# samuel-vitorino/lm.rs

Measured on AMD Instinct MI355X. Metric: decode tok/s + %HBM-roofline, Llama-3.2-1B Q8_0 @1/2/4/8 MI355X vs CPU ref, higher is better.
Workload: dtype int8xint8->int32, f32 combine; 1 GPU; llama-3.2-1b Q8_0 (gs=128) greedy decode, 5-token synthetic prompt then 3164 tokens, batch 1; parallelism=single GPU, image_bytes=1274634496

## Files before the change

lm.rs_amd/csrc/lmrs_kernels.hip:

```cpp
#include <hip/hip_ext.h>
#include <mutex>
#include <map>
#include <set>
#include <tuple>
#include <utility>

#include "lmrs_device_math.h"
#include "lmrs_kernels.h"
#include "lmrs_stage.h"

namespace lmrs {

constexpr int kBlock = 256;
constexpr int kGS = 128;


constexpr int kMaxP = 16;

template <int NP>
__device__ __forceinline__ void rmsnorm_inplace(float4 (&v)[NP], const float4 (&wv)[NP], int n, float eps,
                                                int add_unit, float* scratch) {
    const int t = threadIdx.x;
    const int P = (n + 1023) >> 10;
    const int JP = (n >> 3) + 4;
// ... 1155 lines not shown
    }
    for (int j = tid; j < (ROT ? 0 : half); j += kBlock) {
        float2 cs;
        if constexpr (PRE) cs = pre.cs; else if constexpr (TAG) cs = cs_tag; else cs = *reinterpret_cast<const float2*>(a.rope + ((size_t)pos * half + j) * 2);
        const float fcr = cs.x, fci = cs.y;
        const float q0 = TAG ? q[j] : PRE ? pre.q0 : ld_f32<COH>(a.q + h * HS + j), q1 = TAG ? q[j + half] : PRE ? pre.q1 : ld_f32<COH>(a.q + h * HS + j + half);
        const float2 rq = rope_rotate(q0, q1, fcr, fci);
        q[j] = rq.x; q[j + half] = rq.y;
        const float k0 = TAG ? kn[j] : PRE ? pre.k0 : ld_f32<COH>(a.k_raw + kvh * HS + j), k1 = TAG ? kn[j + half] : PRE ? pre.k1 : ld_f32<COH>(a.k_raw + kvh * HS + j + half);
        const float2 rk = rope_rotate(k0, k1, fcr, fci);
        kn[j] = rk.x; kn[j + half] = rk.y;
        k_store_pair(kT, S, pos, j, half, rk.x, rk.y);
        if constexpr (COH) {
            vn[j] = ld_f32<true>(vbase + (size_t)pos * kv_dim + j);
            vn[j + half] = ld_f32<true>(vbase + (size_t)pos * kv_dim + j + half);
        }
    }
    if (!TAG || HS / 4 > KG || T > kBlock) asm volatile("s_waitcnt vmcnt(0)" ::: "memory");
    lds_barrier();
    ATT_STAMP(2);
    if (!ROT && tc0 == pos) {
#pragma unroll
        for (int u = 0; u < KG; ++u) { const float4 t4 = reinterpret_cast<const float4*>(kn)[u]; kk[u] = f32x4v{t4.x, t4.y, t4.z, t4.w}; }
    }

    int wpos = pos;
    if constexpr (GEMMA) { const int wb = a.st->win_base; wpos = wb >= 0 ? wb : pos; }
    const float sqrt_hs = sqrtf((float)HS);
    float lmax = __uint_as_float(0xff800000u);
    auto finish_score = [&](float score, int t) __attribute__((always_inline)) {
        score = score / sqrt_hs;
        if constexpr (GEMMA) score = gemma_cap_window(score, wpos, t);
        if (t < T) { att[t] = score; lmax = fmaxf(lmax, score); }
    };
    finish_score(att_score_chain<HS, KG>(kk, krs, tc0 * 16, q, S), tid);
    for (int t0 = kBlock; t0 < T; t0 += kBlock) {
        const int t = t0 + tid, tc = t < T ? t : T - 1;
        f32x4v k0[KG];
        att_kload<KG>(k0, krs, tc * 16, 0, S);
        finish_score(att_score_chain<HS, KG>(k0, krs, tc * 16, q, S), t);
    }
    ATT_STAMP(4);
    lmax = wave64_max(lmax);
    if ((tid & 63) == 0) red[tid >> 6] = lmax;
    lds_barrier();
    const float mx = fmaxf(fmaxf(red[0], red[1]), fmaxf(red[2], red[3]));
    for (int t0 = 0; t0 < T; t0 += kBlock) {
        const int t = t0 + tid;
        const float e = expf_glibc_t(t < T ? att[t] - mx : 0.0f, etab);
        if (t < T) att[t] = e;
    }
    if (tid < 64) att[T + tid] = 0.0f;
    lds_barrier();
    if (tid < 64) {
        float sum = 0.0f;
        for (int t0 = 0; t0 < T; t0 += 64) {
            const int left = T - t0;
            sum = wave_serial_sum(sum, att[t0 + tid], left >= 64 ? 4 : (left + 15) >> 4);
        }
        if (tid == 0) red[4] = sum;
    }
    lds_barrier();
    const float sum = red[4];
    for (int t = tid; t < T; t += kBlock) att[t] = att[t] / sum;
    lds_barrier();
    ATT_STAMP(5);

    float o = 0.0f;
    for (int c = 0; c < nchunks; ++c) {
        const int t0 = c * CH, ct = (T - t0) < CH ? (T - t0) : CH;
        att_tstore<HS, NF, true>(vreg, tile, att + t0, t0, T, CH, (COH || TAG) ? pos : -1, vn);
        lds_barrier();
        if (c + 1 < nchunks) att_gload<HS, NF>(vreg, vbase, t0 + CH, T, CH, kv_dim);
        if (c == 0) ATT_STAMP(6);
        if (tid < HS) {
            o = serial_sum16<RS, false>(o, tile + tid, ct);
        }
        lds_barrier();
    }
    if (tid < HS) st_f32<COH>(a.out + h * HS + tid, o);
    ATT_STAMP(7);
}

template <int HS, bool GEMMA>
__global__ __launch_bounds__(kBlock) void attention_kernel(const AttnArgs a) {
    extern __shared__ __attribute__((aligned(16))) char smem[];
    const int h = blockIdx.x, kvh = h / (a.n_heads / a.n_kv_heads);
    ATT_STAMP(0);
    const uint64_t etab = exp2f_tab_lane();
    constexpr int half = HS / 2;
    const int j = threadIdx.x < half ? (int)threadIdx.x : 0;
    const int pos = a.st->pos;
    AttPre pre;
    pre.q0 = a.q[h * HS + j]; pre.q1 = a.q[h * HS + j + half];
    pre.k0 = a.k_raw[kvh * HS + j]; pre.k1 = a.k_raw[kvh * HS + j + half];
    pre.cs = *reinterpret_cast<const float2*>(a.rope + ((size_t)pos * half + j) * 2);
    ATT_STAMP(1);
    attention_body<HS, kAttF4, false, true, GEMMA>(a, h, pos, smem, etab, pre);
}

static size_t attention_smem(int head_size, int chunk, int seq_len) {
    return (size_t)(3 * head_size + 16 + (size_t)(chunk + 32) * (head_size + 4) + ((seq_len + 3) & ~3) + 64) * 4;
}

int attention_chunk(int head_size) {
    int ch = (16384 / head_size) & ~31;
    if (ch > 256) ch = 256;
    return ch < 32 ? 32 : ch;
}

template <int HS, bool GEMMA>
static hipError_t launch_attention_hsg(const AttnArgs& a, size_t smem, hipStream_t s) {
    allow_big_lds(reinterpret_cast<const void*>(attention_kernel<HS, GEMMA>));
    LMRS_LAUNCH_GRID((attention_kernel<HS, GEMMA>), dim3(a.n_heads), kBlock, smem, s, a);
    return hipGetLastError();
}
template <int HS>
static hipError_t launch_attention_hs(const AttnArgs& a, size_t smem, hipStream_t s) {
    return a.gemma ? launch_attention_hsg<HS, true>(a, smem, s) : launch_attention_hsg<HS, false>(a, smem, s);
}

hipError_t launch_attention(const AttnArgs& a0, hipStream_t s) {
    AttnArgs a = a0;
    a.chunk = attention_chunk(a.head_size);
    if (a.chunk * (a.head_size / 4) > kAttF4 * kBlock) return hipErrorInvalidValue;
    const size_t smem = attention_smem(a.head_size, a.chunk, a.seq_len);
    switch (a.head_size) {
        case 64: return launch_attention_hs<64>(a, smem, s);
        case 96: return launch_attention_hs<96>(a, smem, s);
        case 128: return launch_attention_hs<128>(a, smem, s);
        case 256: return launch_attention_hs<256>(a, smem, s);
        default: return hipErrorInvalidValue;
    }
}

template <int HS> struct WaveGeom {
    static constexpr int HS4 = HS / 4, ND = (HS + 63) / 64, NH2 = (HS / 2 + 63) / 64;
    static constexpr int TW = HS <= 64 ? 128 : 64;
    static constexpr int NPASS = TW / 64;
    static constexpr size_t SMEM = (size_t)(2 * HS + TW + 16) * 4 + (size_t)HS4 * TW * 16;
};
constexpr int qa_wave_T(int hs) { return hs == 64 ? 64 * 4 : ((hs == 96 || hs == 128) ? 128 : 0); }

template <int HS, bool GEMMA>
__device__ __forceinline__ void attention_wave_tag(const AttnArgs& a, const int h, const int pos, char* smem, const uint64_t etab, const AttTag& tg) {
    using W = WaveGeom<HS>;
    constexpr int HS4 = W::HS4, ND = W::ND, NH2 = W::NH2, TW = W::TW, NPASS = W::NPASS, half = HS / 2;
    const int lane = threadIdx.x & 63;
    const int kv_mul = a.n_heads / a.n_kv_heads, kvh = h / kv_mul, kv_dim = a.n_kv_heads * HS;
    const int T = pos + 1, S = a.seq_len;
    float* qs = reinterpret_cast<float*>(smem);
    float* kn = qs + HS;
    float* att = kn + HS;
    float4* kt = reinterpret_cast<float4*>(att + TW + 16);
    float* kT = att_k_head(a, kvh, HS);
    const float* vbase = a.v_cache + (size_t)a.layer * S * kv_dim + kvh * HS;
    if (a.dbg && lane == 0 && blockIdx.x == 0) a.dbg[0] = wall_clock64();

    float2 cs[NH2];
#pragma unroll
    for (int i = 0; i < NH2; ++i) { const int j = lane + 64 * i; cs[i] = *reinterpret_cast<const float2*>(a.rope + ((size_t)pos * half + (j < half ? j : 0)) * 2); }
#pragma unroll
    for (int p = 0; p < NPASS; ++p) {
        if (64 * p < pos) {
#pragma unroll
            for (int g = 0; g < HS4; ++g)
                __builtin_amdgcn_global_load_lds((const LMRS_GLOBAL void*)(kT + ((size_t)g * S + 64 * p + lane) * 4),
                                                 (__attribute__((address_space(3))) void*)(kt + g * TW + 64 * p), 16, 0, 0);
        }
    }
    float v[ND][TW];
    const __amdgpu_buffer_rsrc_t vrs = __builtin_amdgcn_make_buffer_rsrc(const_cast<float*>(vbase), 0, 0x7fffffff, 0x00020000);
    const int vrow = kv_dim * 4;
    auto vblock = [&](auto self, auto t0c) __attribute__((always_inline)) -> void {
        constexpr int t0 = decltype(t0c)::value;
        if constexpr (t0 < TW) {
            if (t0 < pos) {
#pragma unroll
                for (int u = 0; u < 16; ++u)
#pragma unroll
                    for (int i = 0; i < ND; ++i) {
                        const int d = lane + 64 * i;
                        v[i][t0 + u] = __uint_as_float(__builtin_amdgcn_raw_buffer_load_b32(vrs, (d < HS ? d : 0) * 4, (t0 + u) * vrow, 0));
                    }
                self(self, std::integral_constant<int, t0 + 16>());
            }
        }
    };
    vblock(vblock, std::integral_constant<int, 0>());
#pragma unroll
    for (int t = 0; t < TW; ++t)
#pragma unroll
        for (int i = 0; i < ND; ++i) { v[i][t] = t < pos ? v[i][t] : 0.0f; asm volatile("" : "+v"(v[i][t])); }
    if (a.dbg && lane == 0 && blockIdx.x == 0) a.dbg[1] = wall_clock64();

    unsigned long long xg[3 * ND];
    {
        const unsigned long long* gp[3 * ND];
#pragma unroll
        for (int i = 0; i < ND; ++i) { const int d = lane + 64 * i; granules_of(tg, h, kvh, HS, d < HS ? d : 0, gp + 3 * i); }
        poll_granules<3 * ND>(gp, tg, a.layer, xg);
    }
    asm volatile("s_waitcnt vmcnt(0)" ::: "memory");
    if (a.dbg && lane == 0 && blockIdx.x == 0) a.dbg[2] = wall_clock64();
    float vnew[ND];
#pragma unroll
    for (int i = 0; i < ND; ++i) {
        const int d = lane + 64 * i;
        vnew[i] = __uint_as_float((unsigned)xg[3 * i + 2]);
        if (d < HS) { qs[d] = __uint_as_float((unsigned)xg[3 * i]); kn[d] = __uint_as_float((unsigned)xg[3 * i + 1]); }
    }
#pragma unroll
    for (int i = 0; i < NH2; ++i) {
        const int j = lane + 64 * i;
        if (j < half) {
            const float2 rq = rope_rotate(qs[j], qs[j + half], cs[i].x, cs[i].y);
            qs[j] = rq.x; qs[j + half] = rq.y;
            const float2 rk = rope_rotate(kn[j], kn[j + half], cs[i].x, cs[i].y);
            k_store_pair(kT, S, pos, j, half, rk.x, rk.y);
            k_store_pair(reinterpret_cast<float*>(kt), TW, pos, j, half, rk.x, rk.y);
        }
    }
    if (a.dbg && lane == 0 && blockIdx.x == 0) a.dbg[3] = wall_clock64();

    int wpos = pos;
    if constexpr (GEMMA) { const int wb = a.st->win_base; wpos = wb >= 0 ? wb : pos; }
    const float sqrt_hs = sqrtf((float)HS), ninf = __uint_as_float(0xff800000u);
    float sc[NPASS];
    float lmax = ninf;
#pragma unroll
    for (int p = 0; p < NPASS; ++p) {
        sc[p] = ninf;
        if (64 * p < T) {
            const int t = 64 * p + lane;
            float score = tile_score<HS4>(kt + t, TW, qs) / sqrt_hs;
            if constexpr (GEMMA) score = gemma_cap_window(score, wpos, t);
            sc[p] = t < T ? score : ninf;
            lmax = fmaxf(lmax, sc[p]);
        }
    }
    if (a.dbg && lane == 0 && blockIdx.x == 0) a.dbg[4] = wall_clock64();
    const float mx = wave64_max(lmax);
    float ex[NPASS];
#pragma unroll
    for (int p = 0; p < NPASS; ++p) {
        ex[p] = 0.0f;
        if (64 * p < T) {
            const int t = 64 * p + lane;
            const float e = expf_glibc_t(t < T ? sc[p] - mx : 0.0f, etab);
            ex[p] = t < T ? e : 0.0f;
        }
    }
    float sum = 0.0f;
#pragma unroll
    for (int p = 0; p < NPASS; ++p) {
        if (64 * p < T) {
            const int left = T - 64 * p;
            sum = wave_serial_sum(sum, ex[p], left >= 64 ? 4 : (left + 15) >> 4);
        }
    }
    float ap_lane = 0.0f;
#pragma unroll
    for (int p = 0; p < NPASS; ++p) {
        if (64 * p < T) {
            const int t = 64 * p + lane;
            const float w = ex[p] / sum;
            att[t] = t < pos ? w : 0.0f;
            if ((pos >> 6) == p) ap_lane = w;
        }
    }
    const float a_pos = __builtin_bit_cast(float, __builtin_amdgcn_readlane(__builtin_bit_cast(int, ap_lane), pos & 63));
    if (a.dbg && lane == 0 && blockIdx.x == 0) a.dbg[5] = wall_clock64();
    float o[ND];
#pragma unroll
    for (int i = 0; i < ND; ++i) o[i] = 0.0f;
#pragma unroll
    for (int t0 = 0; t0 < TW; t0 += 16) {
        if (t0 < pos) {
            float4 w4[4];
#pragma unroll
            for (int u = 0; u < 4; ++u) w4[u] = reinterpret_cast<const float4*>(att)[t0 / 4 + u];
#pragma unroll
            for (int u = 0; u < 4; ++u)
#pragma unroll
                for (int i = 0; i < ND; ++i) {
                    float pr;
                    pr = w4[u].x * v[i][t0 + 4 * u + 0]; o[i] = o[i] + pr;
                    pr = w4[u].y * v[i][t0 + 4 * u + 1]; o[i] = o[i] + pr;
                    pr = w4[u].z * v[i][t0 + 4 * u + 2]; o[i] = o[i] + pr;
                    pr = w4[u].w * v[i][t0 + 4 * u + 3]; o[i] = o[i] + pr;
                }
        }
    }
#pragma unroll
    for (int i = 0; i < ND; ++i) {
        const int d = lane + 64 * i;
        const float pr = a_pos * vnew[i];
        o[i] = o[i] + pr;
        if (d < HS) a.out[h * HS + d] = o[i];
    }
    if (a.dbg && lane == 0 && blockIdx.x == 0) a.dbg[7] = wall_clock64();
}

constexpr size_t kPairSmem = (size_t)(2 * 2 * 64 + 128 + 16 + 16) * 4 + (size_t)16 * 128 * 16 + (size_t)64 * 64 * 4;
template <bool GEMMA>
__device__ __forceinline__ void attention_pair_tag(const AttnArgs& a, const int h, const int pos, char* smem, const uint64_t etab, const AttTag& tg) {
    constexpr int HS = 64, HS4 = 16, TW = 128, half = 32;
    const int lane = threadIdx.x & 63, wv = __builtin_amdgcn_readfirstlane((int)threadIdx.x >> 6);
    const bool two = pos >= 64;
    if (wv > (two ? 1 : 0)) return;
    const int tb = two ? 64 * wv : 0;
    const int kv_mul = a.n_heads / a.n_kv_heads, kvh = h / kv_mul, kv_dim = a.n_kv_heads * HS;
    const int T = pos + 1, S = a.seq_len;
    float* base = reinterpret_cast<float*>(smem);
    float* qs = base + wv * 2 * HS;
    float* kn = qs + HS;
    float* att = base + 4 * HS;
    float* red = att + TW + 16;
    float4* kt = reinterpret_cast<float4*>(red + 16);
    float* prod = reinterpret_cast<float*>(kt + HS4 * TW);
    float* kT = att_k_head(a, kvh, HS);
    const float* vbase = a.v_cache + (size_t)a.layer * S * kv_dim + kvh * HS;
    if (a.dbg && lane == 0 && wv == 0 && blockIdx.x == 0) a.dbg[0] = wall_clock64();

    const float2 cs = *reinterpret_cast<const float2*>(a.rope + ((size_t)pos * half + (lane < half ? lane : 0)) * 2);
    if (tb < pos) {
#pragma unroll
        for (int g = 0; g < HS4; ++g)
            __builtin_amdgcn_global_load_lds((const LMRS_GLOBAL void*)(kT + ((size_t)g * S + tb + lane) * 4),
                                             (__attribute__((address_space(3))) void*)(kt + g * TW + tb), 16, 0, 0);
    }
    float v[64];
    const __amdgpu_buffer_rsrc_t vrs = __builtin_amdgcn_make_buffer_rsrc(const_cast<float*>(vbase), 0, 0x7fffffff, 0x00020000);
    const int vrow = kv_dim * 4, vb0 = tb * vrow;
    auto vblock = [&](auto self, auto u0c) __attribute__((always_inline)) -> void {
        constexpr int u0 = decltype(u0c)::value;
        if constexpr (u0 < 64) {
            if (tb + u0 < pos) {
#pragma unroll
                for (int u = 0; u < 16; ++u) v[u0 + u] = __uint_as_float(__builtin_amdgcn_raw_buffer_load_b32(vrs, lane * 4, vb0 + (u0 + u) * vrow, 0));
                self(self, std::integral_constant<int, u0 + 16>());
            }
        }
    };
    vblock(vblock, std::integral_constant<int, 0>());
#pragma unroll
    for (int u = 0; u < 64; ++u) { v[u] = tb + u < pos ? v[u] : 0.0f; asm volatile("" : "+v"(v[u])); }
    if (a.dbg && lane == 0 && wv == 0 && blockIdx.x == 0) a.dbg[1] = wall_clock64();

    unsigned long long xg[3];
    {
        const unsigned long long* gp[3];
        granules_of(tg, h, kvh, HS, lane, gp);
        poll_granules<3>(gp, tg, a.layer, xg);
    }
    asm volatile("s_waitcnt vmcnt(0)" ::: "memory");
    if (a.dbg && lane == 0 && wv == 0 && blockIdx.x == 0) a.dbg[2] = wall_clock64();
    const float vnew = __uint_as_float((unsigned)xg[2]);
    qs[lane] = __uint_as_float((unsigned)xg[0]); kn[lane] = __uint_as_float((unsigned)xg[1]);
    if (lane < half) {
        const int j = lane;
        const float2 rq = rope_rotate(qs[j], qs[j + half], cs.x, cs.y);
        qs[j] = rq.x; qs[j + half] = rq.y;
        const float2 rk = rope_rotate(kn[j], kn[j + half], cs.x, cs.y);
        if (wv == 0) k_store_pair(kT, S, pos, j, half, rk.x, rk.y);
        if ((pos >> 6) == (two ? wv : 0)) k_store_pair(reinterpret_cast<float*>(kt), TW, pos, j, half, rk.x, rk.y);
    }
    if (a.dbg && lane == 0 && wv == 0 && blockIdx.x == 0) a.dbg[3] = wall_clock64();

    int wpos = pos;
    if constexpr (GEMMA) { const int wb = a.st->win_base; wpos = wb >= 0 ? wb : pos; }
    const float sqrt_hs = sqrtf((float)HS), ninf = __uint_as_float(0xff800000u);
    const int t = tb + lane;
    float sc;
    {
        float score = tile_score<HS4>(kt + t, TW, qs) / sqrt_hs;
        if constexpr (GEMMA) score = gemma_cap_window(score, wpos, t);
        sc = t < T ? score : ninf;
    }
    if (a.dbg && lane == 0 && wv == 0 && blockIdx.x == 0) a.dbg[4] = wall_clock64();
    float mx = wave64_max(sc);
    if (two) {
        if (lane == 0) red[wv] = mx;
        lds_barrier();
        mx = fmaxf(red[0], red[1]);
    }
    const float e0 = expf_glibc_t(t < T ? sc - mx : 0.0f, etab);
    const float ex = t < T ? e0 : 0.0f;
    float sum;
    if (!two) {
        sum = wave_serial_sum(0.0f, ex, (T + 15) >> 4);
    } else {
        if (wv == 0) { sum = wave_serial_sum(0.0f, ex, 4); if (lane == 0) red[2] = sum; }
        lds_barrier();
        if (wv == 1) { sum = wave_serial_sum(red[2], ex, (T - 64 + 15) >> 4); if (lane == 0) red[3] = sum; }
        lds_barrier();
        sum = red[3];
    }
    const float w = ex / sum;
    att[t] = t < pos ? w : 0.0f;
    const bool own_pos = (pos >> 6) == (two ? wv : 0);
    float a_pos = 0.0f;
    if (own_pos) a_pos = __builtin_bit_cast(float, __builtin_amdgcn_readlane(__builtin_bit_cast(int, w), pos & 63));
    if (a.dbg && lane == 0 && wv == 0 && blockIdx.x == 0) a.dbg[5] = wall_clock64();
    if (two && wv == 1) {
        if (lane == 0) red[4] = a_pos;
#pragma unroll
        for (int u0 = 0; u0 < 64; u0 += 16) {
            if (64 + u0 < pos) {
                float4 w4[4];
#pragma unroll
                for (int u = 0; u < 4; ++u) w4[u] = reinterpret_cast<const float4*>(att)[(64 + u0) / 4 + u];
#pragma unroll
                for (int u = 0; u < 4; ++u) {
                    prod[(u0 + 4 * u + 0) * HS + lane] = w4[u].x * v[u0 + 4 * u + 0];
                    prod[(u0 + 4 * u + 1) * HS + lane] = w4[u].y * v[u0 + 4 * u + 1];
                    prod[(u0 + 4 * u + 2) * HS + lane] = w4[u].z * v[u0 + 4 * u + 2];
                    prod[(u0 + 4 * u + 3) * HS + lane] = w4[u].w * v[u0 + 4 * u + 3];
                }
            }
        }
        lds_barrier();
        return;
    }
    float o = 0.0f;
#pragma unroll
    for (int u0 = 0; u0 < 64; u0 += 16) {
        if (u0 < pos) {
            float4 w4[4];
#pragma unroll
            for (int u = 0; u < 4; ++u) w4[u] = reinterpret_cast<const float4*>(att)[u0 / 4 + u];
#pragma unroll
            for (int u = 0; u < 4; ++u) {
                float pr;
                pr = w4[u].x * v[u0 + 4 * u + 0]; o = o + pr;
                pr = w4[u].y * v[u0 + 4 * u + 1]; o = o + pr;
                pr = w4[u].z * v[u0 + 4 * u + 2]; o = o + pr;
                pr = w4[u].w * v[u0 + 4 * u + 3]; o = o + pr;
            }
        }
    }
    if (two) {
        lds_barrier();
        a_pos = red[4];
#pragma unroll
        for (int u0 = 0; u0 < 64; u0 += 16) {
            if (64 + u0 < pos) {
                float pb[16];
#pragma unroll
                for (int u = 0; u < 16; ++u) pb[u] = prod[(u0 + u) * HS + lane];
#pragma unroll
                for (int u = 0; u < 16; ++u) o = o + pb[u];
            }
        }
    }
    {
        const float pr = a_pos * vnew;
        o = o + pr;
        a.out[h * HS + lane] = o;
    }
    if (a.dbg && lane == 0 && wv == 0 && blockIdx.x == 0) a.dbg[7] = wall_clock64();
}

constexpr int kMultiWaves = 4;
constexpr size_t kMultiSmem = (size_t)(kMultiWaves * 2 * 64 + 64 * kMultiWaves + 16 + 32) * 4 + (size_t)(kMultiWaves - 1) * 64 * 64 * 4;
template <bool GEMMA>
__device__ __forceinline__ void attention_multi_tag(const AttnArgs& a, const int h, const int pos, char* smem, const uint64_t etab, const AttTag& tg) {
    constexpr int HS = 64, HS4 = 16, half = 32;
    const int lane = threadIdx.x & 63, wv = __builtin_amdgcn_readfirstlane((int)threadIdx.x >> 6);
    const int nw = (pos >> 6) + 1 < kMultiWaves ? (pos >> 6) + 1 : kMultiWaves;
    if (wv >= nw) return;
    const int tb = 64 * wv, t = tb + lane;
    const int kv_mul = a.n_heads / a.n_kv_heads, kvh = h / kv_mul, kv_dim = a.n_kv_heads * HS;
    const int T = pos + 1, S = a.seq_len;
    float* base = reinterpret_cast<float*>(smem);
    float* qs = base + wv * 2 * HS;
    float* kn = qs + HS;
    float* att = base + kMultiWaves * 2 * HS;
    float* red = att + 64 * kMultiWaves + 16;
    float* prod = red + 32;
    float* kT = att_k_head(a, kvh, HS);
    const float* vbase = a.v_cache + (size_t)a.layer * S * kv_dim + kvh * HS;
    if (a.dbg && lane == 0 && wv == 0 && blockIdx.x == 0) a.dbg[0] = wall_clock64();

    const float2 cs = *reinterpret_cast<const float2*>(a.rope + ((size_t)pos * half + (lane < half ? lane : 0)) * 2);
    f32x4v kreg[HS4];
    {
        const int tk = t < S ? t : S - 1;
        if (tb < pos) {
#pragma unroll
            for (int g = 0; g < HS4; ++g) kreg[g] = *reinterpret_cast<const f32x4v*>(kT + ((size_t)g * S + tk) * 4);
        } else {
#pragma unroll
            for (int g = 0; g < HS4; ++g) kreg[g] = f32x4v{0.0f, 0.0f, 0.0f, 0.0f};
        }
    }
    float v[64];
    const __amdgpu_buffer_rsrc_t vrs = __builtin_amdgcn_make_buffer_rsrc(const_cast<float*>(vbase), 0, 0x7fffffff, 0x00020000);
    const int vrow = kv_dim * 4;
    auto vblock = [&](auto self, auto u0c) __attribute__((always_inline)) -> void {
        constexpr int u0 = decltype(u0c)::value;
        if constexpr (u0 < 64) {
            if (tb + u0 < pos) {
#pragma unroll
                for (int u = 0; u < 16; ++u) {
                    const int row = tb + u0 + u < S ? tb + u0 + u : S - 1;
                    v[u0 + u] = __uint_as_float(__builtin_amdgcn_raw_buffer_load_b32(vrs, lane * 4, row * vrow, 0));
                }
                self(self, std::integral_constant<int, u0 + 16>());
            }
        }
    };
    vblock(vblock, std::integral_constant<int, 0>());
#pragma unroll
    for (int u = 0; u < 64; ++u) { v[u] = tb + u < pos ? v[u] : 0.0f; asm volatile("" : "+v"(v[u])); }
    if (a.dbg && lane == 0 && wv == 0 && blockIdx.x == 0) a.dbg[1] = wall_clock64();

    unsigned long long xg[3];
    {
        const unsigned long long* gp[3];
        granules_of(tg, h, kvh, HS, lane, gp);
        poll_granules<3>(gp, tg, a.layer, xg);
    }
    asm volatile("s_waitcnt vmcnt(0)" ::: "memory");
    if (a.dbg && lane == 0 && wv == 0 && blockIdx.x == 0) a.dbg[2] = wall_clock64();
    const float vnew = __uint_as_float((unsigned)xg[2]);
    qs[lane] = __uint_as_float((unsigned)xg[0]); kn[lane] = __uint_as_float((unsigned)xg[1]);
    const bool own_pos = (pos >> 6) == wv;
    if (lane < half) {
        const int j = lane;
        const float2 rq = rope_rotate(qs[j], qs[j + half], cs.x, cs.y);
        qs[j] = rq.x; qs[j + half] = rq.y;
        const float2 rk = rope_rotate(kn[j], kn[j + half], cs.x, cs.y);
        kn[j] = rk.x; kn[j + half] = rk.y;
        if (wv == 0) k_store_pair(kT, S, pos, j, half, rk.x, rk.y);
    }
    if (own_pos) {
#pragma unroll
        for (int g = 0; g < HS4; ++g) {
            const float4 n4 = reinterpret_cast<const float4*>(kn)[g];
            const bool me = lane == (pos & 63);
            kreg[g][0] = me ? n4.x : kreg[g][0]; kreg[g][1] = me ? n4.y : kreg[g][1]; kreg[g][2] = me ? n4.z : kreg[g][2]; kreg[g][3] = me ? n4.w : kreg[g][3];
        }
    }
    if (a.dbg && lane == 0 && wv == 0 && blockIdx.x == 0) a.dbg[3] = wall_clock64();

    int wpos = pos;
    if constexpr (GEMMA) { const int wb = a.st->win_base; wpos = wb >= 0 ? wb : pos; }
    const float sqrt_hs = sqrtf((float)HS), ninf = __uint_as_float(0xff800000u);
    float sc;
    {
        float score = 0.0f;
#pragma unroll
        for (int g = 0; g < HS4; ++g) {
            const float4 q4 = reinterpret_cast<const float4*>(qs)[g];
            float pr;
            pr = q4.x * kreg[g][0]; score = score + pr;
            pr = q4.y * kreg[g][1]; score = score + pr;
            pr = q4.z * kreg[g][2]; score = score + pr;
            pr = q4.w * kreg[g][3]; score = score + pr;
        }
        score = score / sqrt_hs;
        if constexpr (GEMMA) score = gemma_cap_window(score, wpos, t);
        sc = t < T ? score : ninf;
    }
    if (a.dbg && lane == 0 && wv == 0 && blockIdx.x == 0) a.dbg[4] = wall_clock64();
    float mx = wave64_max(sc);
    if (nw > 1) {
        if (lane == 0) red[wv] = mx;
        lds_barrier();
        mx = red[0];
        for (int w = 1; w < nw; ++w) mx = fmaxf(mx, red[w]);
    }
    const float e0 = expf_glibc_t(t < T ? sc - mx : 0.0f, etab);
    const float ex = t < T ? e0 : 0.0f;
    float sum;
    if (nw == 1) {
        sum = wave_serial_sum(0.0f, ex, (T + 15) >> 4);
    } else {
        for (int s = 0; s < nw; ++s) {
            if (wv == s) {
                const int left = T - 64 * s;
                const float part = wave_serial_sum(s ? red[8 + s - 1] : 0.0f, ex, left >= 64 ? 4 : (left + 15) >> 4);
                if (lane == 0) red[8 + s] = part;
            }
            lds_barrier();
        }
        sum = red[8 + nw - 1];
    }
    const float w = ex / sum;
    att[t] = t < pos ? w : 0.0f;
    float a_pos = 0.0f;
    if (own_pos) a_pos = __builtin_bit_cast(float, __builtin_amdgcn_readlane(__builtin_bit_cast(int, w), pos & 63));
    if (a.dbg && lane == 0 && wv == 0 && blockIdx.x == 0) a.dbg[5] = wall_clock64();
    if (wv > 0) {
        if (own_pos && lane == 0) red[4] = a_pos;
        float* mine = prod + (size_t)(wv - 1) * 64 * HS;
#pragma unroll
        for (int u0 = 0; u0 < 64; u0 += 16) {
            if (tb + u0 < pos) {
                float4 w4[4];
#pragma unroll
                for (int u = 0; u < 4; ++u) w4[u] = reinterpret_cast<const float4*>(att)[(tb + u0) / 4 + u];
#pragma unroll
                for (int u = 0; u < 4; ++u) {
                    mine[(u0 + 4 * u + 0) * HS + lane] = w4[u].x * v[u0 + 4 * u + 0];
                    mine[(u0 + 4 * u + 1) * HS + lane] = w4[u].y * v[u0 + 4 * u + 1];
                    mine[(u0 + 4 * u + 2) * HS + lane] = w4[u].z * v[u0 + 4 * u + 2];
                    mine[(u0 + 4 * u + 3) * HS + lane] = w4[u].w * v[u0 + 4 * u + 3];
                }
            }
        }
        lds_barrier();
        return;
    }
    float o = 0.0f;
#pragma unroll
    for (int u0 = 0; u0 < 64; u0 += 16) {
        if (u0 < pos) {
            float4 w4[4];
#pragma unroll
            for (int u = 0; u < 4; ++u) w4[u] = reinterpret_cast<const float4*>(att)[u0 / 4 + u];
#pragma unroll
            for (int u = 0; u < 4; ++u) {
                float pr;
                pr = w4[u].x * v[u0 + 4 * u + 0]; o = o + pr;
                pr = w4[u].y * v[u0 + 4 * u + 1]; o = o + pr;
                pr = w4[u].z * v[u0 + 4 * u + 2]; o = o + pr;
                pr = w4[u].w * v[u0 + 4 * u + 3]; o = o + pr;
            }
        }
    }
    if (nw > 1) {
        lds_barrier();
        a_pos = red[4];
        for (int k0 = 0; k0 < 64 * (kMultiWaves - 1); k0 += 16) {
            if (64 + k0 < pos) {
                float pb[16];
#pragma unroll
                for (int u = 0; u < 16; ++u) pb[u] = prod[(k0 + u) * HS + lane];
#pragma unroll
                for (int u = 0; u < 16; ++u) o = o + pb[u];
            }
        }
    }
    {
        const float pr = a_pos * vnew;
        o = o + pr;
        a.out[h * HS + lane] = o;
    }
    if (a.dbg && lane == 0 && wv == 0 && blockIdx.x == 0) a.dbg[7] = wall_clock64();
}

template <int HS> struct QuadGeom {
    static constexpr int HS4 = HS / 4, ND = (HS + 63) / 64, NH2 = (HS / 2 + 63) / 64;
    static constexpr int KPW = HS <= 128 ? 32 : 16, TWK = 4 * KPW;
    static constexpr int NPASS = TWK / 64;
    static constexpr size_t SMEM = (size_t)(4 * 2 * HS + TWK + 16 + 32) * 4 + (size_t)HS4 * TWK * 16;
    static_assert((size_t)3 * KPW * ND * 64 * 4 <= (size_t)HS4 * TWK * 16, "the products alias the K tile");
};
template <int HS, bool GEMMA>
__device__ __forceinline__ void attention_quad_tag(const AttnArgs& a, const int h, const int pos, char* smem, const uint64_t etab, const AttTag& tg) {
    using Q = QuadGeom<HS>;
    constexpr int HS4 = Q::HS4, ND = Q::ND, NH2 = Q::NH2, KPW = Q::KPW, TWK = Q::TWK, half = HS / 2;
    const int lane = threadIdx.x & 63, wv = __builtin_amdgcn_readfirstlane((int)threadIdx.x >> 6);
    const int kpw = (KPW == 32 && pos >= 64) ? 32 : 16;
    const int tb = kpw * wv;
    const int kv_mul = a.n_heads / a.n_kv_heads, kvh = h / kv_mul, kv_dim = a.n_kv_heads * HS;
    const int T = pos + 1, S = a.seq_len;
    float* base = reinterpret_cast<float*>(smem);
    float* qs = base + wv * 2 * HS;
    float* kn = qs + HS;
    float* att = base + 4 * 2 * HS;
    float* red = att + TWK + 16;
    float4* kt = reinterpret_cast<float4*>(red + 32);
    float* prod = reinterpret_cast<float*>(kt);
    float* kT = att_k_head(a, kvh, HS);
    const float* vbase = a.v_cache + (size_t)a.layer * S * kv_dim + kvh * HS;
    if (a.dbg && lane == 0 && wv == 0 && blockIdx.x == 0) a.dbg[0] = wall_clock64();

    float2 cs[NH2];
#pragma unroll
    for (int i = 0; i < NH2; ++i) { const int j = lane + 64 * i; cs[i] = *reinterpret_cast<const float2*>(a.rope + ((size_t)pos * half + (j < half ? j : 0)) * 2); }
#pragma unroll
    for (int p = 0; p < Q::NPASS; ++p) {
        if (64 * p < pos) {
#pragma unroll
            for (int gg = 0; gg < HS4 / 4; ++gg) {
                const int g = wv * (HS4 / 4) + gg;
                __builtin_amdgcn_global_load_lds((const LMRS_GLOBAL void*)(kT + ((size_t)g * S + 64 * p + lane) * 4),
                                                 (__attribute__((address_space(3))) void*)(kt + g * TWK + 64 * p), 16, 0, 0);
            }
        }
    }
    float v[ND][KPW];
    const __amdgpu_buffer_rsrc_t vrs = __builtin_amdgcn_make_buffer_rsrc(const_cast<float*>(vbase), 0, 0x7fffffff, 0x00020000);
    const int vrow = kv_dim * 4, vb0 = tb * vrow;
    auto vblock = [&](auto self, auto u0c) __attribute__((always_inline)) -> void {
        constexpr int u0 = decltype(u0c)::value;
        if constexpr (u0 < KPW) {
            if (u0 < kpw && tb + u0 < pos) {
#pragma unroll
                for (int u = 0; u < 16; ++u)
#pragma unroll
                    for (int i = 0; i < ND; ++i) {
                        const int d = lane + 64 * i;
                        v[i][u0 + u] = __uint_as_float(__builtin_amdgcn_raw_buffer_load_b32(vrs, (d < HS ? d : 0) * 4, vb0 + (u0 + u) * vrow, 0));
                    }
                self(self, std::integral_constant<int, u0 + 16>());
            }
        }
    };
    vblock(vblock, std::integral_constant<int, 0>());
#pragma unroll
    for (int u = 0; u < KPW; ++u)
#pragma unroll
        for (int i = 0; i < ND; ++i) { v[i][u] = (u < kpw && tb + u < pos) ? v[i][u] : 0.0f; asm volatile("" : "+v"(v[i][u])); }
    if (a.dbg && lane == 0 && wv == 0 && blockIdx.x == 0) a.dbg[1] = wall_clock64();

    unsigned long long xg[3 * ND];
    {
        const unsigned long long* gp[3 * ND];
#pragma unroll
        for (int i = 0; i < ND; ++i) { const int d = lane + 64 * i; granules_of(tg, h, kvh, HS, d < HS ? d : 0, gp + 3 * i); }
        poll_granules<3 * ND>(gp, tg, a.layer, xg);
    }
    asm volatile("s_waitcnt vmcnt(0)" ::: "memory");
    if (a.dbg && lane == 0 && wv == 0 && blockIdx.x == 0) a.dbg[2] = wall_clock64();
    float vnew[ND];
#pragma unroll
    for (int i = 0; i < ND; ++i) {
        const int d = lane + 64 * i;
        vnew[i] = __uint_as_float((unsigned)xg[3 * i + 2]);
        if (d < HS) { qs[d] = __uint_as_float((unsigned)xg[3 * i]); kn[d] = __uint_as_float((unsigned)xg[3 * i + 1]); }
    }
#pragma unroll
    for (int i = 0; i < NH2; ++i) {
        const int j = lane + 64 * i;
        if (j < half) {
            const float2 rq = rope_rotate(qs[j], qs[j + half], cs[i].x, cs[i].y);
            qs[j] = rq.x; qs[j + half] = rq.y;
            const float2 rk = rope_rotate(kn[j], kn[j + half], cs[i].x, cs[i].y);
            kn[j] = rk.x; kn[j + half] = rk.y;
            if (wv == 0) k_store_pair(kT, S, pos, j, half, rk.x, rk.y);
        }
    }
    lds_barrier();
    if (a.dbg && lane == 0 && wv == 0 && blockIdx.x == 0) a.dbg[3] = wall_clock64();

    int wpos = pos;
    if constexpr (GEMMA) { const int wb = a.st->win_base; wpos = wb >= 0 ? wb : pos; }
    const float sqrt_hs = sqrtf((float)HS), ninf = __uint_as_float(0xff800000u);
    const bool mine = lane < kpw;
    const int t = tb + (mine ? lane : 0);
    float sc;
    {
        const bool own = t == pos;
        float score = tile_score<HS4>(own ? reinterpret_cast<const float4*>(kn) : kt + t, own ? 1 : TWK, qs) / sqrt_hs;
        if constexpr (GEMMA) score = gemma_cap_window(score, wpos, t);
        sc = (mine && t < T) ? score : ninf;
    }
    if (a.dbg && lane == 0 && wv == 0 && blockIdx.x == 0) a.dbg[4] = wall_clock64();
    float mx = wave64_max(sc);
    if (lane == 0) red[wv] = mx;
    lds_barrier();
    mx = fmaxf(fmaxf(red[0], red[1]), fmaxf(red[2], red[3]));
    const float e0 = expf_glibc_t((mine && t < T) ? sc - mx : 0.0f, etab);
    const float ex = (mine && t < T) ? e0 : 0.0f;
    if (mine) att[t] = ex;
    lds_barrier();
    float sum;
    {
        const float ea = att[lane];
        sum = wave_serial_sum(0.0f, ea, T >= 64 ? 4 : (T + 15) >> 4);
        if constexpr (TWK > 64) {
            if (T > 64) { const float eb = att[64 + lane]; sum = wave_serial_sum(sum, eb, (T - 64 + 15) >> 4); }
        }
    }
    const float w = ex / sum;
    const float wz = (mine && t < pos) ? w : 0.0f;
    const bool own_pos = pos >= tb && pos < tb + kpw;
    if (own_pos) {
        const float ap = __builtin_bit_cast(float, __builtin_amdgcn_readlane(__builtin_bit_cast(int, w), pos - tb));
        if (lane == 0) red[4] = ap;
    }
    if (a.dbg && lane == 0 && wv == 0 && blockIdx.x == 0) a.dbg[5] = wall_clock64();
    if (wv > 0) {
        float* dst = prod + (size_t)(tb - kpw) * ND * 64;
#pragma unroll
        for (int u0 = 0; u0 < KPW; u0 += 16) {
            if (u0 < kpw && tb + u0 < pos) {
#pragma unroll
                for (int u = 0; u < 16; ++u) {
                    const float wt = __builtin_bit_cast(float, __builtin_amdgcn_readlane(__builtin_bit_cast(int, wz), u0 + u));
#pragma unroll
                    for (int i = 0; i < ND; ++i) dst[((u0 + u) * ND + i) * 64 + lane] = wt * v[i][u0 + u];
                }
            }
        }
        lds_barrier();
        return;
    }
    float o[ND];
#pragma unroll
    for (int i = 0; i < ND; ++i) o[i] = 0.0f;
#pragma unroll
    for (int u0 = 0; u0 < KPW; u0 += 16) {
        if (u0 < kpw && u0 < pos) {
#pragma unroll
            for (int u = 0; u < 16; ++u) {
                const float wt = __builtin_bit_cast(float, __builtin_amdgcn_readlane(__builtin_bit_cast(int, wz), u0 + u));
#pragma unroll
                for (int i = 0; i < ND; ++i) { const float pr = wt * v[i][u0 + u]; o[i] = o[i] + pr; }
            }
        }
    }
    lds_barrier();
    const float a_pos = red[4];
    for (int k0 = 0; k0 < 3 * kpw; k0 += 8) {
        if (kpw + k0 < pos) {
            float pb[8][ND];
#pragma unroll
            for (int u = 0; u < 8; ++u)
#pragma unroll
                for (int i = 0; i < ND; ++i) pb[u][i] = prod[((k0 + u) * ND + i) * 64 + lane];
#pragma unroll
            for (int u = 0; u < 8; ++u)
#pragma unroll
                for (int i = 0; i < ND; ++i) o[i] = o[i] + pb[u][i];
        }
    }
#pragma unroll
    for (int i = 0; i < ND; ++i) {
        const int d = lane + 64 * i;
        const float pr = a_pos * vnew[i];
        o[i] = o[i] + pr;
        if (d < HS) a.out[h * HS + d] = o[i];
    }
    if (a.dbg && lane == 0 && wv == 0 && blockIdx.x == 0) a.dbg[7] = wall_clock64();
}

constexpr int qa_chunk(int hs) { return (8192 / hs) & ~31; }
template <int HS> struct QaGeom { static constexpr int CH = qa_chunk(HS), NF = (CH * (HS / 4) + kBlock - 1) / kBlock; };

template <int N, int L, int PRO, bool Q4, int HS, bool GEMMA, bool WAVE>
__global__ __launch_bounds__(kBlock) void qkv_attn_kernel(LMRS_HOT_PARAMS, const QkvAttnArgs a0) {
    extern __shared__ __attribute__((aligned(16))) char smem[];
    QkvAttnArgs a = a0;
    a.g = with_hot(a0.g, h_xin, h_wq, h_ws, h_rms_w, h_st, h_seq, h_out); a.t.st = h_st;
    const int nh = a.t.n_heads;
    if ((int)blockIdx.x < nh) {
        const uint64_t etab = exp2f_tab_lane();
        const int pos = a.t.st->pos;
        const AttTag tg{a.g.gran, *a.g.seq + 1u, a.g.att_dim, a.g.kv_dim, a.err};
        const int nkv = a.t.n_kv_heads, bq = (int)blockIdx.x / nkv, br = (int)blockIdx.x - bq * nkv;
        const int head = br * (nh / nkv) + bq;
        if constexpr (WAVE && HS == 64) { if (pos < 128) attention_pair_tag<GEMMA>(a.t, head, pos, smem, etab, tg); else attention_multi_tag<GEMMA>(a.t, head, pos, smem, etab, tg); }
        else if constexpr (WAVE) {
            if (pos < 64) { if (threadIdx.x >= 64) return; attention_wave_tag<HS, GEMMA>(a.t, head, pos, smem, etab, tg); }
            else attention_quad_tag<HS, GEMMA>(a.t, head, pos, smem, etab, tg);
        }
        else attention_body<HS, QaGeom<HS>::NF, false, false, GEMMA, false, true>(a.t, head, pos, smem, etab, AttPre(), tg);
    } else {
        gemv_static_body<N, L, PRO, EPI_QKV_TAG, kBlock, Q4>(a.g, smem, (int)blockIdx.x - nh, (int)gridDim.x - nh);
    }
}

#define LMRS_QA_TABLE(X)                                                                                                \
    X(2048, 32, PRO_RMS_QUANT, false, 64, false)                                                  \
    X(3072, 32, PRO_RMS_QUANT, false, 128, false)                                                 \
    X(3072, 16, PRO_RMS_QUANT, false, 96, false) X(3072, 32, PRO_RMS_QUANT, false, 96, false)               \
    X(2304, 16, PRO_RMS_QUANT, false, 256, true) X(2304, 16, PRO_ADD_RMS_QUANT, false, 256, true)     \
    X(2304, 8, PRO_RMS_QUANT, true, 256, true) X(2304, 8, PRO_ADD_RMS_QUANT, true, 256, true)         \
    X(2048, 16, PRO_RMS_QUANT, true, 64, false)

bool qkv_attn_supported(const GemvArgs& g, int pro, const AttnArgs& t) {
    const StaticClass sc = static_class(g, pro, EPI_QKV);
    if (!sc.L || sc.nt != kBlock || t.n_heads <= 0) return false;
#define X(n_, l_, p_, q_, hs_, gm_) if (g.n == n_ && sc.L == l_ && pro == p_ && (g.q4 != 0) == q_ && t.head_size == hs_ && (t.gemma != 0) == gm_) return true;
    LMRS_QA_TABLE(X)
#undef X
    return false;
}
int qkv_attn_wave_T(int head_size) { return qa_wave_T(head_size); }

static int resident_grid_cap(const void* fn, size_t smem) {
    static std::mutex mu;
    static std::map<std::tuple<int, const void*, size_t>, int> cache;
    int dev = 0, cus = 0, occ = 0;
    (void)hipGetDevice(&dev);
    std::lock_guard<std::mutex> lock(mu);
    auto it = cache.find({dev, fn, smem});
    if (it != cache.end()) return it->second;
    if (hipDeviceGetAttribute(&cus, hipDeviceAttributeMultiprocessorCount, dev) != hipSuccess || cus <= 0) cus = 256;
    if (hipOccupancyMaxActiveBlocksPerMultiprocessor(&occ, fn, kBlock, smem) != hipSuccess || occ <= 0) { (void)hipGetLastError(); occ = 0; }
    const int cap = occ * cus;
    cache[{dev, fn, smem}] = cap;
    return cap;
}
static int qkv_attn_grid(const void* fn, size_t smem, int grid, int n_heads) {
    const int cap = resident_grid_cap(fn, smem);
    return (cap > n_heads + 64 && grid > cap) ? cap : grid;
}

template <int N, int L, int PRO, bool Q4, int HS, bool GEMMA>
static hipError_t launch_qkv_attn_class(const QkvAttnArgs& a, int grid, size_t gsmem, int max_T, bool wave, hipStream_t s) {
    if constexpr (qa_wave_T(HS) > 0) {
        if (wave) {
            constexpr size_t wsm = HS == 64 ? (kMultiSmem > kPairSmem ? kMultiSmem : kPairSmem) : (QuadGeom<HS>::SMEM > WaveGeom<HS>::SMEM ? QuadGeom<HS>::SMEM : WaveGeom<HS>::SMEM);
            size_t smem = wsm > gsmem ? wsm : gsmem;
            if (smem > 64 * 1024) allow_big_lds(reinterpret_cast<const void*>(qkv_attn_kernel<N, L, PRO, Q4, HS, GEMMA, true>));
            grid = qkv_attn_grid(reinterpret_cast<const void*>(qkv_attn_kernel<N, L, PRO, Q4, HS, GEMMA, true>), smem, grid, a.t.n_heads);
            LMRS_LAUNCH_GRID((qkv_attn_kernel<N, L, PRO, Q4, HS, GEMMA, true>), dim3(grid), kBlock, smem, s, LMRS_HOT_OF(a.g), a);
            return hipGetLastError();
        }
    }
    if (wave) return hipErrorNotSupported;
    size_t smem = attention_smem(HS, qa_chunk(HS), max_T);
    if (gsmem > smem) smem = gsmem;
    if (smem > 64 * 1024) allow_big_lds(reinterpret_cast<const void*>(qkv_attn_kernel<N, L, PRO, Q4, HS, GEMMA, false>));
    grid = qkv_attn_grid(reinterpret_cast<const void*>(qkv_attn_kernel<N, L, PRO, Q4, HS, GEMMA, false>), smem, grid, a.t.n_heads);
    LMRS_LAUNCH_GRID((qkv_attn_kernel<N, L, PRO, Q4, HS, GEMMA, false>), dim3(grid), kBlock, smem, s, LMRS_HOT_OF(a.g), a);
    return hipGetLastError();
}

hipError_t launch_qkv_attn(const GemvArgs& g0, int pro, const AttnArgs& t0, int* err, int max_T, bool wave, hipStream_t s) {
    if (!qkv_attn_supported(g0, pro, t0) || !g0.gran || !g0.seq || !err) return hipErrorNotSupported;
    QkvAttnArgs a{g0, t0, err};
    a.g.order_barrier = a.g.chain_spread = 1;
    a.t.chunk = qa_chunk(t0.head_size);
    const StaticClass sc = static_class(a.g, pro, EPI_QKV);
    const int grid = t0.n_heads + gemv_grid(a.g, pro, EPI_QKV);
    const size_t gsmem = gemv_smem(a.g, pro);
#define X(n_, l_, p_, q_, hs_, gm_)                                                                                      \
    if (a.g.n == n_ && sc.L == l_ && pro == p_ && (a.g.q4 != 0) == q_ && t0.head_size == hs_ && (t0.gemma != 0) == gm_)  \
        return launch_qkv_attn_class<n_, l_, p_, q_, hs_, gm_>(a, grid, gsmem, max_T, wave, s);
    LMRS_QA_TABLE(X)
#undef X
    return hipErrorNotSupported;
}

template <int HS, bool GEMMA>
__global__ __launch_bounds__(kBlock) void attention_split_scores_kernel(const AttnArgs a, float* S) {
    __shared__ __attribute__((aligned(16))) float q[HS];
    __shared__ __attribute__((aligned(16))) float kn[HS];
    constexpr int half = HS / 2;
    const int h = blockIdx.x, tid = threadIdx.x;
// ... 618 lines not shown
```

Measured before the change: 1321 tok/s.

## Replace serial cross-wave softmax sum with redundant per-wave scan and overlap value chain

The softmax denominator in the pair and multi-wave attention paths used to be computed by handing a running sum from wave to wave through LDS, with one barrier per wave. Now every wave writes its exponentials to LDS once, and after a single barrier each wave redundantly recomputes the full serial sum in the same order. The value accumulation in wave 0 now does most of its own products before the barrier and double-buffers the LDS loads of the products parked by the other waves, so barrier and load latency overlap useful work. Optional fine-grained timestamp probes are added but compiled out by default. The cost is extra redundant arithmetic per wave and more LDS traffic.

```diff
diff --git a/lm.rs_amd/csrc/lmrs_kernels.hip b/lm.rs_amd/csrc/lmrs_kernels.hip
--- a/lm.rs_amd/csrc/lmrs_kernels.hip
+++ b/lm.rs_amd/csrc/lmrs_kernels.hip
@@ -1481,6 +1481,84 @@
     if (a.dbg && lane == 0 && blockIdx.x == 0) a.dbg[7] = wall_clock64();
 }
 
+#ifndef LMRS_ATT_FINE
+#define LMRS_ATT_FINE 0
+#endif
+#define ATT_FINE(set, k) do { if constexpr (LMRS_ATT_FINE == (set)) { if (a.dbg && threadIdx.x == 0 && blockIdx.x == 0) a.dbg[k] = wall_clock64(); } } while (0)
+
+template <int NW>
+__device__ __forceinline__ float split_serial_sum(const float ex, float* xs, const int wv, const int nw, const int lane, const int T) {
+    xs[128 * wv + lane] = ex;
+    lds_barrier();
+    float e[NW];
+#pragma unroll
+    for (int s = 1; s < NW; ++s) e[s] = xs[128 * s + lane];
+    float sum;
+    if (wv == 0) sum = wave_serial_sum(0.0f, ex, 4);
+    else sum = wave_serial_sum(0.0f, xs[lane], 4);
+#pragma unroll
+    for (int s = 1; s < NW; ++s) {
+        if (s < nw) {
+            const int left = T - 64 * s;
+            sum = wave_serial_sum(sum, e[s], left >= 64 ? 4 : (left + 15) >> 4);
+        }
+    }
+    return sum;
+}
+
+template <int NBMAX, class Stamp>
+__device__ __forceinline__ float value_chain_own_then_parked(const float* att, const float (&v)[64], const float* parked, const int nb, Stamp stamp) {
+    const float4* a4 = reinterpret_cast<const float4*>(att);
+    float o = 0.0f;
+    auto own = [&](int u) __attribute__((always_inline)) {
+        const float4 w = a4[u];
+        float pr;
+        pr = w.x * v[4 * u + 0]; o = o + pr;
+        pr = w.y * v[4 * u + 1]; o = o + pr;
+        pr = w.z * v[4 * u + 2]; o = o + pr;
+        pr = w.w * v[4 * u + 3]; o = o + pr;
+    };
+#pragma unroll
+    for (int u = 0; u < 12; ++u) own(u);
+    stamp(1);
+    lds_barrier();
+    stamp(3);
+    float A[2][16];
+    if (nb > 0) lds_batch16<64>(A[0], parked);
+    asm volatile("" : "+v"(o) : : "memory");
+#pragma unroll
+    for (int u = 12; u < 16; ++u) own(u);
+    stamp(6);
+#pragma unroll
+    for (int b = 0; b < NBMAX; ++b) {
+        if (b < nb) {
+            if (b + 1 < NBMAX && b + 1 < nb) lds_batch16<64>(A[(b + 1) & 1], parked + (b + 1) * 16 * 64);
+            asm volatile("" : "+v"(o) : : "memory");
+#pragma unroll
+            for (int u = 0; u < 16; ++u) o = o + A[b & 1][u];
+        }
+    }
+    return o;
+}
+
+__device__ __forceinline__ void park_products(const float* att, const float (&v)[64], float* parked, const int nb) {
+    float4 w4[16];
+#pragma unroll
+    for (int u = 0; u < 16; ++u) w4[u] = reinterpret_cast<const float4*>(att)[u];
+#pragma unroll
+    for (int b = 0; b < 4; ++b) {
+        if (b < nb) {
+#pragma unroll
+            for (int u = 4 * b; u < 4 * b + 4; ++u) {
+                parked[(4 * u + 0) * 64] = w4[u].x * v[4 * u + 0];
+                parked[(4 * u + 1) * 64] = w4[u].y * v[4 * u + 1];
+                parked[(4 * u + 2) * 64] = w4[u].z * v[4 * u + 2];
+                parked[(4 * u + 3) * 64] = w4[u].w * v[4 * u + 3];
+            }
+        }
+    }
+}
+
 constexpr size_t kPairSmem = (size_t)(2 * 2 * 64 + 128 + 16 + 16) * 4 + (size_t)16 * 128 * 16 + (size_t)64 * 64 * 4;
 template <bool GEMMA>
 __device__ __forceinline__ void attention_pair_tag(const AttnArgs& a, const int h, const int pos, char* smem, const uint64_t etab, const AttTag& tg) {
@@ -1564,18 +1642,14 @@
         lds_barrier();
         mx = fmaxf(red[0], red[1]);
     }
+    ATT_FINE(1, 1);
     const float e0 = expf_glibc_t(t < T ? sc - mx : 0.0f, etab);
     const float ex = t < T ? e0 : 0.0f;
+    ATT_FINE(1, 3);
     float sum;
-    if (!two) {
-        sum = wave_serial_sum(0.0f, ex, (T + 15) >> 4);
-    } else {
-        if (wv == 0) { sum = wave_serial_sum(0.0f, ex, 4); if (lane == 0) red[2] = sum; }
-        lds_barrier();
-        if (wv == 1) { sum = wave_serial_sum(red[2], ex, (T - 64 + 15) >> 4); if (lane == 0) red[3] = sum; }
-        lds_barrier();
-        sum = red[3];
-    }
+    if (!two) sum = wave_serial_sum(0.0f, ex, (T + 15) >> 4);
+    else sum = split_serial_sum<2>(ex, base + HS, wv, 2, lane, T);
+    ATT_FINE(1, 6);
     const float w = ex / sum;
     att[t] = t < pos ? w : 0.0f;
     const bool own_pos = (pos >> 6) == (two ? wv : 0);
@@ -1584,54 +1658,31 @@
     if (a.dbg && lane == 0 && wv == 0 && blockIdx.x == 0) a.dbg[5] = wall_clock64();
     if (two && wv == 1) {
         if (lane == 0) red[4] = a_pos;
-#pragma unroll
-        for (int u0 = 0; u0 < 64; u0 += 16) {
-            if (64 + u0 < pos) {
-                float4 w4[4];
-#pragma unroll
-                for (int u = 0; u < 4; ++u) w4[u] = reinterpret_cast<const float4*>(att)[(64 + u0) / 4 + u];
-#pragma unroll
-                for (int u = 0; u < 4; ++u) {
-                    prod[(u0 + 4 * u + 0) * HS + lane] = w4[u].x * v[u0 + 4 * u + 0];
-                    prod[(u0 + 4 * u + 1) * HS + lane] = w4[u].y * v[u0 + 4 * u + 1];
-                    prod[(u0 + 4 * u + 2) * HS + lane] = w4[u].z * v[u0 + 4 * u + 2];
-                    prod[(u0 + 4 * u + 3) * HS + lane] = w4[u].w * v[u0 + 4 * u + 3];
-                }
-            }
-        }
+        park_products(att + 64, v, prod + lane, (pos - 64 + 15) >> 4);
         lds_barrier();
         return;
     }
     float o = 0.0f;
-#pragma unroll
-    for (int u0 = 0; u0 < 64; u0 += 16) {
-        if (u0 < pos) {
-            float4 w4[4];
-#pragma unroll
-            for (int u = 0; u < 4; ++u) w4[u] = reinterpret_cast<const float4*>(att)[u0 / 4 + u];
-#pragma unroll
-            for (int u = 0; u < 4; ++u) {
-                float pr;
-                pr = w4[u].x * v[u0 + 4 * u + 0]; o = o + pr;
-                pr = w4[u].y * v[u0 + 4 * u + 1]; o = o + pr;
-                pr = w4[u].z * v[u0 + 4 * u + 2]; o = o + pr;
-                pr = w4[u].w * v[u0 + 4 * u + 3]; o = o + pr;
-            }
-        }
-    }
-    if (two) {
-        lds_barrier();
+    if (!two) {
+#pragma unroll
+        for (int u0 = 0; u0 < 64; u0 += 16) {
+            if (u0 < pos) {
+                float4 w4[4];
+#pragma unroll
+                for (int u = 0; u < 4; ++u) w4[u] = reinterpret_cast<const float4*>(att)[u0 / 4 + u];
+#pragma unroll
+                for (int u = 0; u < 4; ++u) {
+                    float pr;
+                    pr = w4[u].x * v[u0 + 4 * u + 0]; o = o + pr;
+                    pr = w4[u].y * v[u0 + 4 * u + 1]; o = o + pr;
+                    pr = w4[u].z * v[u0 + 4 * u + 2]; o = o + pr;
+                    pr = w4[u].w * v[u0 + 4 * u + 3]; o = o + pr;
+                }
+            }
+        }
+    } else {
+        o = value_chain_own_then_parked<4>(att, v, prod + lane, (pos - 64 + 15) >> 4, [&](int k) __attribute__((always_inline)) { ATT_FINE(2, k); });
         a_pos = red[4];
-#pragma unroll
-        for (int u0 = 0; u0 < 64; u0 += 16) {
-            if (64 + u0 < pos) {
-                float pb[16];
-#pragma unroll
-                for (int u = 0; u < 16; ++u) pb[u] = prod[(u0 + u) * HS + lane];
-#pragma unroll
-                for (int u = 0; u < 16; ++u) o = o + pb[u];
-            }
-        }
     }
     {
         const float pr = a_pos * vnew;
@@ -1751,22 +1802,14 @@
         mx = red[0];
         for (int w = 1; w < nw; ++w) mx = fmaxf(mx, red[w]);
     }
+    ATT_FINE(1, 1);
     const float e0 = expf_glibc_t(t < T ? sc - mx : 0.0f, etab);
     const float ex = t < T ? e0 : 0.0f;
+    ATT_FINE(1, 3);
     float sum;
-    if (nw == 1) {
-        sum = wave_serial_sum(0.0f, ex, (T + 15) >> 4);
-    } else {
-        for (int s = 0; s < nw; ++s) {
-            if (wv == s) {
-                const int left = T - 64 * s;
-                const float part = wave_serial_sum(s ? red[8 + s - 1] : 0.0f, ex, left >= 64 ? 4 : (left + 15) >> 4);
-                if (lane == 0) red[8 + s] = part;
-            }
-            lds_barrier();
-        }
-        sum = red[8 + nw - 1];
-    }
+    if (nw == 1) sum = wave_serial_sum(0.0f, ex, (T + 15) >> 4);
+    else sum = split_serial_sum<kMultiWaves>(ex, base + HS, wv, nw, lane, T);
+    ATT_FINE(1, 6);
     const float w = ex / sum;
     att[t] = t < pos ? w : 0.0f;
     float a_pos = 0.0f;
@@ -1775,53 +1818,31 @@
     if (wv > 0) {
         if (own_pos && lane == 0) red[4] = a_pos;
         float* mine = prod + (size_t)(wv - 1) * 64 * HS;
-#pragma unroll
-        for (int u0 = 0; u0 < 64; u0 += 16) {
-            if (tb + u0 < pos) {
-                float4 w4[4];
-#pragma unroll
-                for (int u = 0; u < 4; ++u) w4[u] = reinterpret_cast<const float4*>(att)[(tb + u0) / 4 + u];
-#pragma unroll
-                for (int u = 0; u < 4; ++u) {
-                    mine[(u0 + 4 * u + 0) * HS + lane] = w4[u].x * v[u0 + 4 * u + 0];
-                    mine[(u0 + 4 * u + 1) * HS + lane] = w4[u].y * v[u0 + 4 * u + 1];
-                    mine[(u0 + 4 * u + 2) * HS + lane] = w4[u].z * v[u0 + 4 * u + 2];
-                    mine[(u0 + 4 * u + 3) * HS + lane] = w4[u].w * v[u0 + 4 * u + 3];
-                }
-            }
-        }
+        park_products(att + tb, v, mine + lane, (pos - tb + 15) >> 4 < 4 ? (pos - tb + 15) >> 4 : 4);
         lds_barrier();
         return;
     }
     float o = 0.0f;
-#pragma unroll
-    for (int u0 = 0; u0 < 64; u0 += 16) {
-        if (u0 < pos) {
-            float4 w4[4];
-#pragma unroll
-            for (int u = 0; u < 4; ++u) w4[u] = reinterpret_cast<const float4*>(att)[u0 / 4 + u];
-#pragma unroll
-            for (int u = 0; u < 4; ++u) {
-                float pr;
-                pr = w4[u].x * v[u0 + 4 * u + 0]; o = o + pr;
-                pr = w4[u].y * v[u0 + 4 * u + 1]; o = o + pr;
-                pr = w4[u].z * v[u0 + 4 * u + 2]; o = o + pr;
-                pr = w4[u].w * v[u0 + 4 * u + 3]; o = o + pr;
-            }
-        }
-    }
-    if (nw > 1) {
-        lds_barrier();
+    if (nw == 1) {
+#pragma unroll
+        for (int u0 = 0; u0 < 64; u0 += 16) {
+            if (u0 < pos) {
+                float4 w4[4];
+#pragma unroll
+                for (int u = 0; u < 4; ++u) w4[u] = reinterpret_cast<const float4*>(att)[u0 / 4 + u];
+#pragma unroll
+                for (int u = 0; u < 4; ++u) {
+                    float pr;
+                    pr = w4[u].x * v[u0 + 4 * u + 0]; o = o + pr;
+                    pr = w4[u].y * v[u0 + 4 * u + 1]; o = o + pr;
+                    pr = w4[u].z * v[u0 + 4 * u + 2]; o = o + pr;
+                    pr = w4[u].w * v[u0 + 4 * u + 3]; o = o + pr;
+                }
+            }
+        }
+    } else {
+        o = value_chain_own_then_parked<4 * (kMultiWaves - 1)>(att, v, prod + lane, (pos - 64 + 15) >> 4, [&](int k) __attribute__((always_inline)) { ATT_FINE(2, k); });
         a_pos = red[4];
-        for (int k0 = 0; k0 < 64 * (kMultiWaves - 1); k0 += 16) {
-            if (64 + k0 < pos) {
-                float pb[16];
-#pragma unroll
-                for (int u = 0; u < 16; ++u) pb[u] = prod[(k0 + u) * HS + lane];
-#pragma unroll
-                for (int u = 0; u < 16; ++u) o = o + pb[u];
-            }
-        }
     }
     {
         const float pr = a_pos * vnew;
```

New measurement: 1323 tok/s, median of 6. Within noise of the previous version (+0.2%).
